# refresh-bio/vclust

Measured on AMD Instinct MI355X. Metric: genome pairs/sec through prefilter+align (ani.tsv), higher is better.
Workload: dtype u64

## Files before the change

### vclust_amd/build.py

```python
import os
import pathlib
import shutil
import subprocess
import sys

PKG_DIR = pathlib.Path(__file__).resolve().parent
ROOT = PKG_DIR.parent
CSRC = PKG_DIR / 'csrc'
LIB_PATH = PKG_DIR / 'libvclust_gpu.so'
ORACLE_DIR = ROOT / 'oracle'

SOURCES = ['vg_core.cpp', 'vg_genomes.cpp', 'vg_inflate.cpp', 'vg_io.cpp', 'vg_api.cpp', 'vg_synth.cpp', 'vg_prefilter.hip', 'vg_align.hip', 'vg_dist.hip', 'vg_cluster.hip', 'vg_dedup.hip']


def _hipcc() -> str:
    for cand in (os.environ.get('HIPCC'), shutil.which('hipcc'), '/opt/rocm/bin/hipcc'):
        if cand and pathlib.Path(cand).exists():
            return cand
    raise RuntimeError('hipcc not found (needs ROCm)')


def _stale(target: pathlib.Path, deps) -> bool:
    if not target.exists():
        return True
    t = target.stat().st_mtime
    return any(pathlib.Path(d).stat().st_mtime > t for d in deps)


def build_lib(force: bool = False, verbose: bool = False) -> pathlib.Path:
    srcs = [CSRC / s for s in SOURCES]
    deps = srcs + [CSRC / 'vg_common.h', ROOT / 'include' / 'vclust_gpu.h']
    if not force and not _stale(LIB_PATH, deps):
        return LIB_PATH
    obj_dir = PKG_DIR / '_obj'
    obj_dir.mkdir(exist_ok=True)
    hipcc = _hipcc()
    flags = ['--offload-arch=gfx950', '-O3', '-std=c++17', '-fPIC', '-Wall', '-Wno-unused-function',
             '-Wno-unused-result', f'-I{ROOT / "include"}']
    if os.environ.get('VG_LINES') == '1':
        flags.append('-gline-tables-only')
    if os.environ.get('VG_DEV') == '1':
        flags.append('-DVG_DEV_KERNELS')
    objs = []
    procs = []
    for s in srcs:
        o = obj_dir / (s.name + '.o')
        objs.append(o)
        if force or _stale(o, [s, CSRC / 'vg_common.h', ROOT / 'include' / 'vclust_gpu.h']):
            cmd = [hipcc, *flags, '-x', 'hip', '-c', str(s), '-o', str(o)]
            if verbose:
                print(' '.join(cmd), file=sys.stderr)
            procs.append((s, subprocess.Popen(cmd, stdout=subprocess.PIPE, stderr=subprocess.STDOUT, text=True)))
    for s, p in procs:
        out, _ = p.communicate()
        if p.returncode != 0:
            raise RuntimeError(f'hipcc failed on {s.name}:\n{out}')
        if verbose and out.strip():
            print(out, file=sys.stderr)
    cmd = [hipcc, '--offload-arch=gfx950', '-shared', '-fPIC', '-o', str(LIB_PATH), *map(str, objs), '-lz', '-lpthread', '-ldl']
    r = subprocess.run(cmd, stdout=subprocess.PIPE, stderr=subprocess.STDOUT, text=True)
    if r.returncode != 0:
        raise RuntimeError(f'link failed:\n{r.stdout}')
    return LIB_PATH


def build_oracle(verbose: bool = False) -> pathlib.Path:
    r = subprocess.run(['make', '-C', str(ORACLE_DIR)], stdout=subprocess.PIPE, stderr=subprocess.STDOUT, text=True)
    if r.returncode != 0:
        raise RuntimeError(f'oracle build failed:\n{r.stdout}')
    if verbose:
        print(r.stdout, file=sys.stderr)
    return ORACLE_DIR / '_build' / 'liboracle.so'


if __name__ == '__main__':
    force = '--force' in sys.argv
    print(build_lib(force=force, verbose=True))
    print(build_oracle(verbose=False))
```

### vclust_amd/csrc/vg_align.hip

```cpp
#include "vg_common.h"
#include <rocprim/rocprim.hpp>
#include <algorithm>
#include <numeric>
#include <cstring>
#include <memory>
#include <mutex>
#include <optional>

namespace {

constexpr int RR_PAD = 128;

struct ref_desc {
    int64_t rr_w;
    int64_t mask_w;
    int64_t stab;
    int64_t sent;
    int32_t L;
    int32_t n_rr;
    int32_t genome;
    int32_t has_n;
    int32_t pos_bits;
    int32_t tag_bits;
};

struct lz_dev_params { int mal, msl, mrd, mqd, reg, aw, am, ar; int ablate; int pw_after, pw_miss; int weak_ratio; int margin; int seed_choice; };


__device__ __forceinline__ uint32_t loadm32(const uint32_t* __restrict__ mk, int64_t p) {
    int64_t w = p >> 5; int sh = (int)(p & 31);
    uint64_t m = (uint64_t)mk[w] | ((uint64_t)mk[w + 1] << 32);
    return (uint32_t)(m >> sh);
}
__device__ __forceinline__ uint32_t squeeze16(uint32_t x) {
    x &= 0x55555555u;
    x = (x | (x >> 1)) & 0x33333333u;
    x = (x | (x >> 2)) & 0x0F0F0F0Fu;
    x = (x | (x >> 4)) & 0x00FF00FFu;
    return (x | (x >> 8)) & 0x0000FFFFu;
}
__device__ __forceinline__ uint32_t squeeze(uint64_t x) {
    return squeeze16((uint32_t)x) | (squeeze16((uint32_t)(x >> 32)) << 16);
}
struct planes32 { uint32_t lo, hi; };
__device__ __forceinline__ planes32 planes_of(uint64_t codes) { return { squeeze(codes), squeeze(codes >> 1) }; }

__device__ __forceinline__ planes32 loadp(const uint32_t* __restrict__ pl, int64_t p) {
    const uint32_t off = ((uint32_t)p >> 5) << 3; const uint32_t sh = (uint32_t)p & 31u;
    uint4 v; __builtin_memcpy(&v, (const char*)pl + off, 16);
    asm volatile("" :: "v"(v.w));
    return { __builtin_amdgcn_alignbit(v.z, v.x, sh), __builtin_amdgcn_alignbit(v.w, v.y, sh) };
}
__device__ __forceinline__ uint32_t diff32(const planes32 a, const planes32 b) { return (a.lo ^ b.lo) | (a.hi ^ b.hi); }
__device__ __forceinline__ uint32_t slots(int lo, int hi) {
    if (lo < 0) lo = 0; if (hi > 32) hi = 32;
    if (hi <= lo) return 0u;
    const uint32_t a = (hi == 32) ? ~0u : ((1u << hi) - 1u);
    return a & ~((1u << lo) - 1u);
}

struct pair_ctx {
    const uint32_t* qpl; const uint32_t* qmk; int qlen; int q_has_n;
    const uint32_t* rpl; const uint32_t* rmk; int n_rr; int L; int r_has_n;
};

__device__ __forceinline__ uint32_t mism32(const pair_ctx& c, int qp, int rp, int rlo, int rhi) {
    const int lo = max(-qp, rlo - rp); const int hi = min(c.qlen - qp, rhi - rp);
    if (lo <= 0 && hi >= 32) {
        uint32_t mm = diff32(loadp(c.qpl, qp), loadp(c.rpl, rp));
        if (c.q_has_n) mm |= loadm32(c.qmk, qp);
        if (c.r_has_n) mm |= loadm32(c.rmk, rp);
        return mm;
    }
    const uint32_t ok = slots(lo, hi);
    if (ok == 0) return ~0u;
    const int qs = qp < 0 ? 0 : qp, rs = rp < 0 ? 0 : rp;
    planes32 xq = loadp(c.qpl, qs), xr = loadp(c.rpl, rs);
    if (qp < 0) { xq.lo <<= -qp; xq.hi <<= -qp; }
    if (rp < 0) { xr.lo <<= -rp; xr.hi <<= -rp; }
    uint32_t mm = diff32(xq, xr);
    if (c.q_has_n) { uint32_t sp = loadm32(c.qmk, qs); if (qp < 0) sp <<= -qp; mm |= sp; }
    if (c.r_has_n) { uint32_t sp = loadm32(c.rmk, rs); if (rp < 0) sp <<= -rp; mm |= sp; }
    return mm | ~ok;
}
__device__ __forceinline__ int strand_lo(const pair_ctx& c, int rp) { return rp > c.L ? c.L + 1 : 0; }
__device__ __forceinline__ int strand_hi(const pair_ctx& c, int rp) { return rp > c.L ? c.n_rr : c.L; }

__device__ __forceinline__ int match_len_lane(const pair_ctx& c, int qp, int rp, int cap) {
    int l = 0;
    while (l < cap) {
        const uint32_t mm = mism32(c, qp + l, rp + l, strand_lo(c, rp), strand_hi(c, rp));
        if (mm) return l + __builtin_ctz(mm);
        l += 32;
    }
    return l;
}

__device__ __forceinline__ int match_len32_q(const pair_ctx& c, const planes32 xq, uint32_t qbad, int rp) {
    uint32_t mm = diff32(xq, loadp(c.rpl, rp)) | qbad;
    if (c.r_has_n) mm |= loadm32(c.rmk, rp);
    const int hi = c.n_rr - rp; if (hi < 32) mm |= ~slots(0, hi);
    const int sj = c.L - rp; if ((unsigned)sj < 32u) mm |= 1u << sj;
    return mm ? __builtin_ctz(mm) : 32;
}

__device__ __forceinline__ uint32_t lane32(uint32_t v, int src_lane) { return (uint32_t)__builtin_amdgcn_readlane((int)v, src_lane); }
__device__ __forceinline__ uint32_t lane_prev32(uint32_t v) {
    return (uint32_t)__builtin_amdgcn_update_dpp(0, (int)v, 0x138, 0xf, 0xf, false);
}
__device__ __forceinline__ int wave_sum(int v) {
    int t = 0;
#pragma unroll
    for (int b = 0; b < 6; ++b) t += __popcll(__ballot((v >> b) & 1)) << b;
    return t;
}

__device__ __forceinline__ uint32_t extend_mask0(const pair_ctx& c, int qp, int rp, int dir, int bound, int lane, int rlo, int rhi) {
    uint32_t mm = ~0u;
    const int e0 = 32 * lane;
    if (e0 < bound) {
        if (dir > 0) mm = mism32(c, qp + e0, rp + e0, rlo, rhi);
        else mm = __brev(mism32(c, qp - e0 - 32, rp - e0 - 32, rlo, rhi));
        const int rem = bound - e0; if (rem < 32) mm |= ~slots(0, rem);
    }
    return mm;
}

__device__ __forceinline__ int extend(const pair_ctx& c, const lz_dev_params& P, int qp, int rp, int dir, int bound,
                                      int lane, int* n_match, uint32_t mm_first, int rlo, int rhi) {
    int accepted = 0, matches_total = 0;
    int first_mm = -1;
    uint32_t carry_mm = 0;
    uint32_t carry_ok = 0;
    int base = 0;
    int cum_before = 0;
    const uint32_t awmask = (P.aw >= 32) ? ~0u : ((1u << P.aw) - 1u);
    if (bound <= 0) { *n_match = 0; return 0; }
    for (;;) {
        uint32_t mm = mm_first;
        if (base > 0) {
            mm = ~0u;
            const int e0 = base + 32 * lane;
            if (e0 < bound) {
                if (dir > 0) mm = mism32(c, qp + e0, rp + e0, rlo, rhi);
                else mm = __brev(mism32(c, qp - e0 - 32, rp - e0 - 32, rlo, rhi));
                const int rem = bound - e0; if (rem < 32) mm |= ~slots(0, rem);
            }
        }
        const unsigned long long anyb = __ballot(mm != 0);
        if (first_mm < 0 && anyb) {
            const int fl = __builtin_ctzll(anyb);
            first_mm = base + 32 * fl + __builtin_ctz(lane32(mm, fl));
        }
        uint32_t prev_mm = lane_prev32(mm); const uint32_t okb = ~mm; uint32_t prev_ok = lane_prev32(okb);
        if (lane == 0) { prev_mm = carry_mm; prev_ok = carry_ok; }
        int viol = 32;
        {
            const uint32_t tail = (P.aw > 1) ? (prev_mm >> (32 - (P.aw - 1))) : 0u;
            if ((int)(__popc(mm) + __popc(tail)) > P.am) {
                uint32_t bits = mm;
                for (int skip = P.am - (int)__popc(tail); skip > 0; --skip) bits &= bits - 1;
                while (bits) {
                    const int j = __builtin_ctz(bits);
                    const uint32_t hi = (j == 31) ? mm : (mm & ((2u << j) - 1u));
                    int cnt;
                    if (j + 1 >= P.aw) cnt = __popc(hi & (awmask << (j + 1 - P.aw)));
                    else cnt = __popc(hi) + __popc(prev_mm >> (32 - (P.aw - 1 - j)));
                    if (cnt > P.am) { viol = j; break; }
                    bits &= bits - 1;
                }
            }
        }
        const unsigned long long vb = __ballot(viol < 32);
        if (anyb) {
            uint32_t run = okb;
            for (int t = 1; t < P.ar; ++t) run &= __builtin_amdgcn_alignbit(okb, prev_ok, (uint32_t)(32 - t));
            const int fv = vb ? __builtin_ctzll(vb) : 64;
            const int vj = (int)lane32((uint32_t)viol, fv & 63);
            uint32_t cand = run;
            if (lane > fv) cand = 0;
            else if (lane == fv) cand &= (vj == 0) ? 0u : ((1u << vj) - 1u);
            const unsigned long long cb = __ballot(cand != 0);
            if (cb) {
                const int hl = 63 - __builtin_clzll(cb);
                const uint32_t ch = lane32(cand, hl); const uint32_t mh = lane32(mm, hl);
                const int hj = 31 - __builtin_clz(ch);
                accepted = base + 32 * hl + hj + 1;
                int tot = wave_sum(lane < hl ? 32 - __popc(mm) : 0);
                const uint32_t upto = (hj == 31) ? ~0u : ((2u << hj) - 1u);
                tot += (hj + 1) - __popc(mh & upto);
                matches_total = cum_before + tot;
            }
        } else {
            accepted = base + 2048; matches_total = cum_before + 2048;
        }
        if (vb) break;
        if (base + 2048 >= bound) break;
        cum_before += anyb ? wave_sum(32 - __popc(mm)) : 2048;
        carry_mm = lane32(mm, 63); carry_ok = lane32(okb, 63);
        base += 2048;
    }
    if (first_mm < 0) first_mm = bound;
    if (first_mm > bound) first_mm = bound;
    if (accepted < first_mm) { accepted = first_mm; matches_total = first_mm; }
    if (accepted > bound) { accepted = bound; }
    *n_match = matches_total;
    return accepted;
}

__device__ __forceinline__ uint64_t low_bits64(int n) { return n >= 64 ? ~0ULL : (n <= 0 ? 0ULL : ((1ULL << n) - 1)); }

__device__ __forceinline__ int gap_score(const pair_ctx& c, int i, int g, int pred0, int E, int lane, int rlo, int rhi,
                                         int* pm_out, int* sm_out) {
    const int reflen = E - pred0;
    const int skip = (reflen >= 0 && g > reflen) ? g - reflen : 0;
    const int q0 = i - g;
    uint32_t ok_o = 0, ok_n = 0;
    {
        const int e0 = 32 * lane;
        if (e0 < g) {
            const uint32_t in = (g - e0 >= 32) ? 0xffffffffu : ((1u << (g - e0)) - 1u);
            ok_o = ~mism32(c, q0 + e0, pred0 + e0, rlo, rhi) & in;
            ok_n = ~mism32(c, q0 + e0, E - g + e0, rlo, rhi) & in;
        }
    }
    int tot_n = 0;
    for (int w2 = 0; 32 * w2 < g; ++w2) tot_n += __popc(lane32(ok_n, w2));
    int best_v = -1, best_pm = 0, best_sm = 0;
    const int nbits = 32 - __builtin_clz((unsigned)g | 1u);
    int po = 0;
    const int n_split = g - skip;
    for (int w = 0; 64 * w <= n_split; ++w) {
        const uint64_t O = (uint64_t)lane32(ok_o, 2 * w) | ((uint64_t)lane32(ok_o, (2 * w + 1) & 63) << 32);
        const int a = 64 * w + lane;
        const int s0 = 64 * w + skip;
        const int ws = s0 >> 6;
        const uint64_t N0 = (uint64_t)lane32(ok_n, (2 * ws) & 63) | ((uint64_t)lane32(ok_n, (2 * ws + 1) & 63) << 32);
        const uint64_t N1 = (uint64_t)lane32(ok_n, (2 * ws + 2) & 63) | ((uint64_t)lane32(ok_n, (2 * ws + 3) & 63) << 32);
        int pn0 = 0;
        for (int w2 = 0; w2 < 2 * ws && 32 * w2 < g; ++w2) pn0 += __popc(lane32(ok_n, w2));
        const int pn1 = pn0 + __popcll(N0);
        const int sp = s0 + lane;
        const bool second = (sp >> 6) > ws;
        const int before = second ? pn1 + __popcll(N1 & low_bits64(sp & 63)) : pn0 + __popcll(N0 & low_bits64(sp & 63));
        const int pre = po + __popcll(O & low_bits64(lane));
        const int suf = tot_n - before;
        const bool valid = a <= n_split;
        const int v = pre + suf;
        unsigned long long act = __ballot(valid);
        if (act) {
            for (int b = nbits - 1; b >= 0; --b) {
                const unsigned long long m = __ballot(valid && ((v >> b) & 1)) & act;
                if (m) act = m;
            }
            const int wl = 63 - __builtin_clzll(act);
            const int vmax = (int)lane32((uint32_t)v, wl);
            if (vmax >= best_v) { best_v = vmax; best_pm = (int)lane32((uint32_t)pre, wl); best_sm = (int)lane32((uint32_t)suf, wl); }
        }
        po += __popcll(O);
    }
    *pm_out = best_pm; *sm_out = best_sm;
    return best_pm + best_sm;
}

__device__ __forceinline__ void rr_chunk_planes(const uint32_t* __restrict__ gpl, const uint32_t* __restrict__ gmk, int L, int64_t ch,
                                                uint32_t* lo_out, uint32_t* hi_out, uint32_t* mask_out) {
    const int64_t p0 = ch * 32;
    uint32_t lo = 0, hi = 0, mask = 0xffffffffu;
    const int64_t nf = (int64_t)L - p0;
    if (nf > 0) {
        const uint32_t xl = gpl[2 * ch], xh = gpl[2 * ch + 1], m = gmk[ch];
        if (nf >= 32) { lo = xl; hi = xh; mask = m; }
        else { const uint32_t lowm = (1u << nf) - 1u; lo = xl & lowm; hi = xh & lowm; mask = (m & lowm) | ~lowm; }
    }
    const int64_t jlo = (L + 1 - p0) > 0 ? (L + 1 - p0) : 0;
    const int64_t jhi = (2 * (int64_t)L - p0) < 31 ? (2 * (int64_t)L - p0) : 31;
    if (jlo <= jhi) {
        const int64_t fstart = 2 * (int64_t)L - p0 - 31;
        planes32 x; uint32_t m;
        if (fstart >= 0) { x = loadp(gpl, fstart); m = loadm32(gmk, fstart); }
        else { x = loadp(gpl, 0); x.lo <<= -fstart; x.hi <<= -fstart; m = loadm32(gmk, 0) << (-fstart); }
        const uint32_t rl = ~__brev(x.lo), rh = ~__brev(x.hi), mr = __brev(m);
        const uint32_t hi1 = (jhi == 31) ? 0xffffffffu : ((1u << (jhi + 1)) - 1);
        const uint32_t lo1 = (jlo == 0) ? 0u : ((1u << jlo) - 1);
        const uint32_t sl1 = hi1 & ~lo1;
        lo |= rl & sl1; hi |= rh & sl1;
        mask = (mask & ~sl1) | (mr & sl1);
    }
    *lo_out = lo & ~mask; *hi_out = hi & ~mask; *mask_out = mask;
}

__device__ __forceinline__ uint32_t bucket_of(uint32_t xl, uint32_t xh, int msl) { const uint32_t m = (1u << msl) - 1u; return (xl & m) | ((xh & m) << msl); }
__device__ __forceinline__ uint32_t tag_of(uint32_t xl, uint32_t xh, int msl, int tag_bits) {
    const int tl = (tag_bits + 1) >> 1, th = tag_bits >> 1;
    return ((xl >> msl) & ((1u << tl) - 1u)) | (((xh >> msl) & ((1u << th) - 1u)) << tl);
}

constexpr int LDS_TAB = 16384;
constexpr int LDS_STAGE = 22016;
constexpr int TOP_BITS = 9;
constexpr int BIG_RR = 131072;
__device__ __forceinline__ void lds_sync() { asm volatile("s_waitcnt lgkmcnt(0)\n\ts_barrier" ::: "memory"); }

__device__ __forceinline__ uint32_t wave_scan_inclusive(uint32_t v) {
    v += (uint32_t)__builtin_amdgcn_update_dpp(0, (int)v, 0x111, 0xf, 0xf, true);
    v += (uint32_t)__builtin_amdgcn_update_dpp(0, (int)v, 0x112, 0xf, 0xf, true);
    v += (uint32_t)__builtin_amdgcn_update_dpp(0, (int)v, 0x114, 0xf, 0xf, true);
    v += (uint32_t)__builtin_amdgcn_update_dpp(0, (int)v, 0x118, 0xf, 0xf, true);
    v += (uint32_t)__builtin_amdgcn_update_dpp(0, (int)v, 0x142, 0xa, 0xf, false);
    v += (uint32_t)__builtin_amdgcn_update_dpp(0, (int)v, 0x143, 0xc, 0xf, false);
    return v;
}
// ... 616 lines not shown
                    }
                    const unsigned long long at = chunk_base + (kk & (RCHUNK - 1));
                    if (lane == 0 && at < arena_cap) {
                        region_rec rg; rg.task = tk.out_idx; rg.qstart = r_qstart; rg.qend = r_qend;
                        rg.rstart = r_rstart; rg.rend = r_rend; rg.n_match = r_match; rg.k = kk; rg.t = (uint32_t)t;
                        arena[at] = rg;
                    }
                }
            }
            in_region = false;
        }
    };

    for (int phase = 0; phase < (S > 1 ? 2 : 1); ++phase) {
    while (i < phase_end) {
        const int qi = i + lane;
        int best_len = 0, best_pos = 0; bool hit_close = false;
        if (qi < lim && lane < pw) {
            const bool alive_l = alive && (lit + lane <= P.mqd);
            const int pred_l = pred + lane;
            const planes32 xq = loadp(c.qpl, qi);
            bool q_ok_a = true, q_ok_s = (qi + P.msl <= c.qlen);
            uint32_t qbad = (c.qlen - qi < 32) ? ~slots(0, c.qlen - qi) : 0u;
            if (c.q_has_n) {
                const uint32_t m = loadm32(c.qmk, qi);
                q_ok_a = (m & ((1u << P.mal) - 1u)) == 0;
                q_ok_s = q_ok_s && (m & ((1u << P.msl) - 1u)) == 0;
                qbad |= m;
            }
            const bool do_a = q_ok_a && !(ABL & 16);
            const bool do_s = alive_l && q_ok_s && !(ABL & 1);
            uint32_t s_u = 0, s_e = 0;
            const uint32_t posmask = (rd.pos_bits >= 32) ? 0xffffffffu : ((1u << rd.pos_bits) - 1u);
            const uint32_t qtag = tag_of(xq.lo, xq.hi, P.msl, rd.tag_bits);
            const bool probing = (do_a || do_s) && q_ok_s;
            const uint32_t b = bucket_of(xq.lo, xq.hi, P.msl);
            uint4 f0 = make_uint4(~0u, ~0u, ~0u, ~0u), f1 = f0;
            if (FUSED) {
                if (probing) { const uint32_t* sl = fslots + ((size_t)tk.r_slot * FUSED_SLOTS + b) * 8; __builtin_memcpy(&f0, sl, 16); __builtin_memcpy(&f1, sl + 4, 16); }
            } else if (probing) {
                uint2 bb; __builtin_memcpy(&bb, stab + (b ? b - 1 : 0u), 8);
                s_u = b ? bb.x : 0u; s_e = b ? bb.y : bb.x;
            }
            const int pred0 = pred - lit;
            const bool pred_rc = pred0 > c.L;
            const int win_lo = pred0;
            const int win_hi = pred_rc ? pred_l + P.mrd - 1 : min(pred_l + P.mrd - 1, c.L - 1);
            int sbest_len = 0, sbest_pos = 0, sbest_ad = 0, ncap_a = 0, ncap_s = 0;
            const uint32_t win_span = (uint32_t)(win_hi - win_lo);
            const bool win_any = win_hi >= win_lo;
            auto scan4 = [&](const uint4 v, const unsigned vm) {
                const uint32_t e4[4] = { v.x, v.y, v.z, v.w };
                unsigned am = 0, sm = 0;
#pragma unroll
                for (int j = 0; j < 4; ++j) {
                    const uint32_t ps = e4[j] & posmask;
                    am |= (uint32_t)(rd.tag_bits == 0 || (e4[j] >> rd.pos_bits) == qtag) << j;
                    sm |= (uint32_t)(ps - (uint32_t)win_lo <= win_span) << j;
                }
                am &= do_a ? vm : 0u; sm &= (do_s && win_any) ? vm : 0u;
                unsigned cm = am | sm;
                while (cm) {
                    const int j = __builtin_ctz(cm); cm &= cm - 1;
                    const uint32_t ej = j == 0 ? e4[0] : j == 1 ? e4[1] : j == 2 ? e4[2] : e4[3];
                    const int rp = (int)(ej & posmask);
                    const int l0 = match_len32_q(c, xq, qbad, rp);
                    if ((am >> j) & 1u) {
                        int l = l0;
                        if (l >= P.mal) {
                            if (l >= 32) {
                                if (ncap_a++ > 0 || best_len >= 32) {
                                    l = match_len_lane(c, qi, rp, 1 << 30);
                                    if (best_len == 32) best_len = match_len_lane(c, qi, best_pos, 1 << 30);
                                }
                            }
                            if (l > best_len || (l == best_len && rp < best_pos)) { best_len = l; best_pos = rp; }
                        }
                    }
                    if ((sm >> j) & 1u) {
                        int l = l0;
                        if (l >= P.msl) {
                            if (l >= 32) {
                                if (ncap_s++ > 0 || sbest_len >= 32) {
                                    l = match_len_lane(c, qi, rp, 1 << 30);
                                    if (sbest_len == 32) sbest_len = match_len_lane(c, qi, sbest_pos, 1 << 30);
                                }
                            }
                            const int ad = abs(rp - pred_l);
                            const bool better = P.seed_choice == 1 ? (sbest_len == 0 || ad < sbest_ad || (ad == sbest_ad && (l > sbest_len || (l == sbest_len && rp < sbest_pos))))
                                                                   : (l > sbest_len || (l == sbest_len && (ad < sbest_ad || (ad == sbest_ad && rp < sbest_pos))));
                            if (better) { sbest_len = l; sbest_pos = rp; sbest_ad = ad; }
                        }
                    }
                }
            };
            if (FUSED) {
                if (DEV) { ++n_ab; }
                const unsigned vm0 = (unsigned)(!(f0.x >> 31)) | ((unsigned)(!(f0.y >> 31)) << 1) | ((unsigned)(!(f0.z >> 31)) << 2) | ((unsigned)(!(f0.w >> 31)) << 3);
                const unsigned vm1 = (unsigned)(!(f1.x >> 31)) | ((unsigned)(!(f1.y >> 31)) << 1) | ((unsigned)(!(f1.z >> 31)) << 2) | ((unsigned)(!(f1.w >> 31)) << 3);
                if (vm0) scan4(f0, vm0);
                if (vm1) scan4(f1, vm1);
                if ((f1.w >> 31) && f1.w != ~0u) {
                    s_u = f1.w & 0x7fffffu; const uint32_t cnt = (f1.w >> 23) & 0xffu;
                    if (cnt == 255u) { uint2 bb; __builtin_memcpy(&bb, stab + (b ? b - 1 : 0u), 8); s_e = b ? bb.y : bb.x; }
                    else s_e = s_u + cnt;
                }
                const unsigned long long hit0 = __ballot(best_len > 0 || sbest_len > 0);
                if (hit0 && lane > __builtin_ctzll(hit0)) s_u = s_e;
            }
            while (s_u < s_e) {
                if (DEV) { ++n_ab; }
                uint4 v; __builtin_memcpy(&v, sent + s_u, 16);
                const uint32_t left = s_e - s_u;
                scan4(v, left >= 4u ? 0xfu : ((1u << left) - 1u));
                s_u += 4;
                const unsigned long long hit = __ballot(best_len > 0 || sbest_len > 0);
                if (hit && lane > __builtin_ctzll(hit)) s_u = s_e;
            }
            if (best_len > 0 && sbest_len > 0 && best_pos != sbest_pos && best_len >= 32 && sbest_len + P.margin + 1 > 32) {
                if (best_len == 32) best_len = match_len_lane(c, qi, best_pos, 1 << 30);
                if (sbest_len == 32) sbest_len = match_len_lane(c, qi, sbest_pos, 1 << 30);
            }
            if (best_len > 0 && (sbest_len == 0 || best_len > sbest_len + P.margin - ((P.weak_ratio > 0 && lit + lane > P.weak_ratio * sbest_len) ? 1 : 0))) {
                const int d = best_pos - pred_l;
                hit_close = alive_l && ((best_pos > c.L) == pred_rc) && d >= -P.mrd && d <= P.mrd;
            } else if (sbest_len > 0) { best_len = sbest_len; best_pos = sbest_pos; hit_close = true; }
        }
        const unsigned long long hb = __ballot(best_len > 0);
        if (DEV) ++n_iter;
        PROF_MARK(0);
        if (!hb) {
            const int n = min(pw, lim - i);
            i += n; lit += n; if (alive) { pred += n; if (lit > P.mqd) alive = false; }
            pw = pw < P.pw_miss ? P.pw_miss : 64;
            continue;
        }
        const int f = __builtin_ctzll(hb);
        pw = P.pw_after;
        if (!(ABL & 64)) {
            ++n_events;
            if (n_events == 24) __builtin_amdgcn_s_setprio(1);
            else if (n_events == 64) __builtin_amdgcn_s_setprio(2);
            else if (n_events == 160) __builtin_amdgcn_s_setprio(3);
        }
        const int ev_pos = (int)lane32((uint32_t)best_pos, f);
        const bool ev_close = lane32((uint32_t)hit_close, f) != 0;
        i += f; lit += f; if (alive) { pred += f; if (lit > P.mqd) alive = false; }
        const int gap_end_ref = pred - 1;
        const int ev_i = i;
        const int ev_len = (int)lane32((uint32_t)best_len, f);
        const int rlo = strand_lo(c, ev_pos), rhi = strand_hi(c, ev_pos);
        const int kept_after = (in_region && r_qend - r_qstart + 1 >= P.reg) ? r_qend + 1 : kept_end;
        const int bwd_bound = ev_close ? 0 : i - kept_after;
        const uint32_t mm_b = (!ev_close && !(ABL & 2)) ? extend_mask0(c, i, ev_pos, -1, bwd_bound, lane, rlo, rhi) : ~0u;
        const uint32_t mm_f = extend_mask0(c, i, ev_pos, +1, 1 << 30, lane, rlo, rhi);
        PROF_MARK(1);
        if (!ev_close) {
            close_region();
            int bm = 0;
            const int b = (ABL & 2) ? 0 : extend(c, P, i, ev_pos, -1, bwd_bound, lane, &bm, mm_b, rlo, rhi);
            r_qstart = i - b; r_rstart = ev_pos - b; r_match = bm; r_rend = -1;
            in_region = true;
        }
        PROF_MARK(2);
        int fe, fm = 0;
        {
            fe = (ABL & 4) ? P.mal : extend(c, P, i, ev_pos, +1, 1 << 30, lane, &fm, mm_f, rlo, rhi);
            r_match += fm;
        }
        if (ev_close) {
            int pm = 0, sm = 0;
            if (lit > 0 && !(ABL & 8)) {
                int xl = ev_len;
                if (xl >= 32) {
                    const unsigned long long mb = __ballot(mm_f != 0);
                    xl = mb ? 32 * __builtin_ctzll(mb) + __builtin_ctz(lane32(mm_f, __builtin_ctzll(mb))) : 2048;
                    if (xl >= 2048) xl = match_len_lane(c, i, ev_pos, 1 << 30);
                }
                r_match += gap_score(c, i, lit, pred - lit, ev_pos + xl, lane, rlo, rhi, &pm, &sm);
            }
            const int tru = gap_end_ref + 1, vir = vend + lit - pm;
            vend = max(tru, vir) - sm + (fe - fm);
            r_rend = max(r_rend, max(ev_pos + fe - 1, vend - 1));
            r_rstart = min(r_rstart, ev_pos);
        }
        i += fe; pred = ev_pos + fe; lit = 0; alive = true;
        if (!ev_close) { r_rend = pred - 1; vend = pred; }
        PROF_MARK(3);
        r_qend = i - 1;
        if (S > 1) {
            const bool span_ok = i - r_qstart >= P.reg;
            if (phase == 1) {
                const int v = min(S - 1, ev_i / seg_len);
                if (v != look_v) { look_v = v; look_cur = 0; }
                const seg_rec* lg = s_log + v * SEG_LOG_CAP; const int nv = s_cnt[v];
                while (look_cur < nv && lg[look_cur].i_ev < ev_i) ++look_cur;
                if (span_ok && look_cur < nv && lg[look_cur].i_ev == ev_i && lg[look_cur].ev_pos == ev_pos && (lg[look_cur].VN >> 31)) {
                    synced = true; sync_v = v; sync_idx = look_cur;
                    M += (uint32_t)r_match; A -= (uint32_t)r_qstart;
                    break;
                }
            } else if (log_n < SEG_LOG_CAP) {
                if (lane == 0) {
                    seg_rec rc; rc.i_ev = ev_i; rc.ev_pos = ev_pos;
                    rc.VM = M + (uint32_t)r_match; rc.VA = A - (uint32_t)r_qstart; rc.VN = NR | (span_ok ? 0x80000000u : 0u);
                    s_log[w * SEG_LOG_CAP + log_n] = rc;
                }
                ++log_n;
            }
        }
    }
    if (S > 1 && phase == 0) {
        if (lane == 0) s_cnt[w] = log_n;
        __syncthreads();
        phase_end = lim;
    }
    if (synced) break;
    }
    if (!synced) close_region();
    if (S > 1) {
        if (lane == 0) { s_end[w][0] = M; s_end[w][1] = A; s_end[w][2] = NR; s_sync_v[w] = sync_v; s_sync_idx[w] = sync_idx; }
        __syncthreads();
        if (threadIdx.x == 0) {
            uint32_t tm = 0, ta = 0, tn = 0, bm = 0, ba = 0, bn = 0; int cur = 0;
            for (;;) {
                tm += s_end[cur][0] - bm; ta += s_end[cur][1] - ba; tn += s_end[cur][2] - bn;
                const int v = s_sync_v[cur];
                if (v < 0) break;
                const seg_rec rc = s_log[v * SEG_LOG_CAP + s_sync_idx[cur]];
                bm = rc.VM; ba = rc.VA; bn = rc.VN & 0x7fffffffu; cur = v;
            }
            vg_pair_stat st; st.n_match = tm; st.aln_len = ta; st.n_regions = tn;
            stats[tk.out_idx] = st;
        }
        return;
    }
    if (prof) { M = (uint32_t)(pc[psel] >> 4); A = (uint32_t)n_events; }
    if (ABL & 1024) {
        int mab = n_ab, msb = n_sb;
        for (int o = 32; o; o >>= 1) { mab = max(mab, __shfl_xor(mab, o)); msb = max(msb, __shfl_xor(msb, o)); }
        M = (uint32_t)n_iter; A = (uint32_t)n_events; if (ABL & 2048) { M = (uint32_t)mab; A = (uint32_t)msb; }
    }
    if (ABL & (32 | 1024)) NR = (uint32_t)((long long)wall_clock64() - t_start);
    if (REG && (NR & (RCHUNK - 1)) != 0) {
        const uint32_t used = NR & (RCHUNK - 1);
        const unsigned long long at = chunk_base + used + (uint32_t)lane;
        if (used + (uint32_t)lane < (uint32_t)RCHUNK && at < arena_cap) arena[at].task = ~0u;
    }
    if (lane == 0) { vg_pair_stat st; st.n_match = M; st.aln_len = A; st.n_regions = NR; stats[tk.out_idx] = st; }
}

#define PARSE_KERNEL(NAME, S, DEV, WAVES, FAST, REG, ...) \
    __global__ void __launch_bounds__(256) __attribute__((amdgpu_waves_per_eu(WAVES, 8))) NAME(PARSE_ARGS) { \
        lz_parse_body<S, DEV, FAST, REG, ##__VA_ARGS__>(PARSE_ARG_NAMES); }
PARSE_KERNEL(k_lz_parse, 1, false, 8, false, false)
PARSE_KERNEL(k_lz_parse_fast, 1, false, 8, true, false)
PARSE_KERNEL(k_lz_parse_seg, 4, false, 8, false, false)
PARSE_KERNEL(k_lz_parse_seg_fast, 4, false, 8, true, false)
PARSE_KERNEL(k_lz_parse_regions, 1, false, 8, false, true)
PARSE_KERNEL(k_lz_parse_fast_regions, 1, false, 8, true, true)
PARSE_KERNEL(k_lz_parse_fast_fused, 1, false, 8, true, false, true)
__global__ void __launch_bounds__(256)
k_index_fuse(const ref_desc* __restrict__ refs, int first_ref, int n_refs, const uint32_t* __restrict__ stab_pool, const uint32_t* __restrict__ sent_pool,
             uint32_t* __restrict__ fslots) {
    for (int r = blockIdx.x; r < n_refs; r += gridDim.x) {
        const ref_desc rd = refs[first_ref + r];
        const uint32_t* stab = stab_pool + rd.stab; const uint32_t* sent = sent_pool + rd.sent;
        uint32_t* out = fslots + (size_t)(first_ref + r) * FUSED_SLOTS * 8;
        for (int b = threadIdx.x; b < FUSED_SLOTS; b += blockDim.x) {
            const uint32_t lo = b ? stab[b - 1] : 0u, hi = stab[b], n = hi - lo;
            uint32_t w[8];
#pragma unroll
            for (int j = 0; j < 8; ++j) w[j] = (uint32_t)j < n ? sent[lo + j] : ~0u;
            if (n > 8) w[7] = 0x80000000u | (((n - 7) < 255u ? (n - 7) : 255u) << 23) | (lo + 7);
            uint4 a = make_uint4(w[0], w[1], w[2], w[3]), c2 = make_uint4(w[4], w[5], w[6], w[7]);
            __builtin_memcpy(out + (size_t)b * 8, &a, 16); __builtin_memcpy(out + (size_t)b * 8 + 4, &c2, 16);
        }
    }
}
#ifdef VG_DEV_KERNELS
PARSE_KERNEL(k_lz_parse_dev, 1, true, 3, false, false)
#endif

__global__ void __launch_bounds__(256)
k_region_counts(const task_dev* __restrict__ tasks, int64_t n_tasks, const vg_pair_stat* __restrict__ stats, unsigned long long* __restrict__ cnt) {
    for (int64_t t = (int64_t)blockIdx.x * blockDim.x + threadIdx.x; t <= n_tasks; t += (int64_t)gridDim.x * blockDim.x)
        cnt[t] = t < n_tasks ? (unsigned long long)stats[tasks[t].out_idx].n_regions : 0ULL;
}
__global__ void __launch_bounds__(256)
k_regions_place(const region_rec* __restrict__ arena, unsigned long long n_slots, const unsigned long long* __restrict__ first,
                unsigned long long n_out, vg_region* __restrict__ out, unsigned int* __restrict__ bad) {
    for (unsigned long long i = (unsigned long long)blockIdx.x * blockDim.x + threadIdx.x; i < n_slots; i += (unsigned long long)gridDim.x * blockDim.x) {
        const region_rec r = arena[i];
        if (r.task == ~0u) continue;
        const unsigned long long at = first[r.t] + r.k;
        if (at >= first[r.t + 1] || at >= n_out) { atomicAdd(bad, 1u); continue; }
        vg_region o; o.task = r.task; o.qstart = r.qstart; o.qend = r.qend; o.rstart = r.rstart; o.rend = r.rend; o.n_match = r.n_match;
        out[at] = o;
    }
}

inline int grid_for(int64_t n, int block = 256, int max_blocks = 256 * 16) {
    int64_t b = (n + block - 1) / block; if (b < 1) b = 1;
    return (int)std::min<int64_t>(b, max_blocks);
}

}

static std::mutex g_fit_mu;
static bool g_fit_set = false;
static vg_lz_fit g_fit{ 3, -1, 3 };
static vg_lz_fit lz_fit_now() {
    std::lock_guard<std::mutex> lk(g_fit_mu);
    if (!g_fit_set) {
        g_fit_set = true;
        if (const char* e = vg_dev_getenv("VG_LZ_WEAK_SEED")) if (*e) g_fit.weak_seed_ratio = atoi(e);
        if (const char* e = vg_dev_getenv("VG_LZ_ANCHOR_MARGIN")) if (*e) g_fit.anchor_margin = atoi(e);
        if (const char* e = vg_dev_getenv("VG_LZ_SEED_CHOICE")) if (*e) g_fit.seed_choice = atoi(e);
        if (g_fit.weak_seed_ratio != 3 || g_fit.anchor_margin >= 0 || g_fit.seed_choice != 3)
            fprintf(stderr, "libvclust_gpu: LZ fit constants changed by developer switches (weak seed ratio %d, anchor margin %d, seed choice %d): results differ from the reference's\n",
// ... 636 lines not shown
```

Measured before the change: 2.550 million.

## Add fast extension path with wide mismatch loads and bit-sliced window check

```diff
diff --git a/vclust_amd/build.py b/vclust_amd/build.py
--- a/vclust_amd/build.py
+++ b/vclust_amd/build.py
@@ -29,7 +29,7 @@
 
 def build_lib(force: bool = False, verbose: bool = False) -> pathlib.Path:
     srcs = [CSRC / s for s in SOURCES]
-    deps = srcs + [CSRC / 'vg_common.h', ROOT / 'include' / 'vclust_gpu.h']
+    deps = srcs + [CSRC / 'vg_common.h', CSRC / 'vg_window.h', ROOT / 'include' / 'vclust_gpu.h']
     if not force and not _stale(LIB_PATH, deps):
         return LIB_PATH
     obj_dir = PKG_DIR / '_obj'
@@ -46,7 +46,7 @@
     for s in srcs:
         o = obj_dir / (s.name + '.o')
         objs.append(o)
-        if force or _stale(o, [s, CSRC / 'vg_common.h', ROOT / 'include' / 'vclust_gpu.h']):
+        if force or _stale(o, [s, CSRC / 'vg_common.h', CSRC / 'vg_window.h', ROOT / 'include' / 'vclust_gpu.h']):
             cmd = [hipcc, *flags, '-x', 'hip', '-c', str(s), '-o', str(o)]
             if verbose:
                 print(' '.join(cmd), file=sys.stderr)
diff --git a/vclust_amd/csrc/vg_align.hip b/vclust_amd/csrc/vg_align.hip
--- a/vclust_amd/csrc/vg_align.hip
+++ b/vclust_amd/csrc/vg_align.hip
@@ -1,4 +1,5 @@
 #include "vg_common.h"
+#include "vg_window.h"
 #include <rocprim/rocprim.hpp>
 #include <algorithm>
 #include <numeric>
@@ -115,9 +116,22 @@
     return t;
 }
 
-__device__ __forceinline__ uint32_t extend_mask0(const pair_ctx& c, int qp, int rp, int dir, int bound, int lane, int rlo, int rhi) {
+template <bool UNI>
+__device__ __forceinline__ uint32_t extend_mask(const pair_ctx& c, int qp, int rp, int dir, int base, int bound, int lane, int rlo, int rhi) {
+    if (UNI && base + 2048 <= bound) {
+        const int q0 = dir > 0 ? qp + base : qp - base - 2048, r0 = dir > 0 ? rp + base : rp - base - 2048;
+        if (q0 >= 0 && q0 + 2048 <= c.qlen && r0 >= rlo && r0 + 2048 <= rhi) {
+            const uint32_t off = (uint32_t)(dir > 0 ? lane : 63 - lane) * 8u;
+            const char* qrow = (const char*)c.qpl + (size_t)(q0 >> 5) * 8; const char* rrow = (const char*)c.rpl + (size_t)(r0 >> 5) * 8;
+            const uint32_t qsh = (uint32_t)q0 & 31u, rsh = (uint32_t)r0 & 31u;
+            uint4 vq, vr; __builtin_memcpy(&vq, qrow + off, 16); __builtin_memcpy(&vr, rrow + off, 16);
+            const uint32_t mm = (__builtin_amdgcn_alignbit(vq.z, vq.x, qsh) ^ __builtin_amdgcn_alignbit(vr.z, vr.x, rsh)) |
+                                (__builtin_amdgcn_alignbit(vq.w, vq.y, qsh) ^ __builtin_amdgcn_alignbit(vr.w, vr.y, rsh));
+            return dir > 0 ? mm : __brev(mm);
+        }
+    }
     uint32_t mm = ~0u;
-    const int e0 = 32 * lane;
+    const int e0 = base + 32 * lane;
     if (e0 < bound) {
         if (dir > 0) mm = mism32(c, qp + e0, rp + e0, rlo, rhi);
         else mm = __brev(mism32(c, qp - e0 - 32, rp - e0 - 32, rlo, rhi));
@@ -125,7 +139,12 @@
     }
     return mm;
 }
-
+template <bool UNI>
+__device__ __forceinline__ uint32_t extend_mask0(const pair_ctx& c, int qp, int rp, int dir, int bound, int lane, int rlo, int rhi) {
+    return extend_mask<UNI>(c, qp, rp, dir, 0, bound, lane, rlo, rhi);
+}
+
+template <bool FAST>
 __device__ __forceinline__ int extend(const pair_ctx& c, const lz_dev_params& P, int qp, int rp, int dir, int bound,
                                       int lane, int* n_match, uint32_t mm_first, int rlo, int rhi) {
     int accepted = 0, matches_total = 0;
@@ -138,15 +157,7 @@
     if (bound <= 0) { *n_match = 0; return 0; }
     for (;;) {
         uint32_t mm = mm_first;
-        if (base > 0) {
-            mm = ~0u;
-            const int e0 = base + 32 * lane;
-            if (e0 < bound) {
-                if (dir > 0) mm = mism32(c, qp + e0, rp + e0, rlo, rhi);
-                else mm = __brev(mism32(c, qp - e0 - 32, rp - e0 - 32, rlo, rhi));
-                const int rem = bound - e0; if (rem < 32) mm |= ~slots(0, rem);
-            }
-        }
+        if (base > 0) mm = extend_mask<FAST>(c, qp, rp, dir, base, bound, lane, rlo, rhi);
         const unsigned long long anyb = __ballot(mm != 0);
         if (first_mm < 0 && anyb) {
             const int fl = __builtin_ctzll(anyb);
@@ -157,7 +168,9 @@
         int viol = 32;
         {
             const uint32_t tail = (P.aw > 1) ? (prev_mm >> (32 - (P.aw - 1))) : 0u;
-            if ((int)(__popc(mm) + __popc(tail)) > P.am) {
+            if ((int)(__popc(mm) + __popc(tail)) > P.am && FAST) {
+                viol = vg_first_violation_15_7(mm, prev_mm);
+            } else if ((int)(__popc(mm) + __popc(tail)) > P.am) {
                 uint32_t bits = mm;
                 for (int skip = P.am - (int)__popc(tail); skip > 0; --skip) bits &= bits - 1;
                 while (bits) {
@@ -1080,20 +1093,20 @@
         const int rlo = strand_lo(c, ev_pos), rhi = strand_hi(c, ev_pos);
         const int kept_after = (in_region && r_qend - r_qstart + 1 >= P.reg) ? r_qend + 1 : kept_end;
         const int bwd_bound = ev_close ? 0 : i - kept_after;
-        const uint32_t mm_b = (!ev_close && !(ABL & 2)) ? extend_mask0(c, i, ev_pos, -1, bwd_bound, lane, rlo, rhi) : ~0u;
-        const uint32_t mm_f = extend_mask0(c, i, ev_pos, +1, 1 << 30, lane, rlo, rhi);
+        const uint32_t mm_b = (!ev_close && !(ABL & 2)) ? extend_mask0<FAST>(c, i, ev_pos, -1, bwd_bound, lane, rlo, rhi) : ~0u;
+        const uint32_t mm_f = extend_mask0<FAST>(c, i, ev_pos, +1, 1 << 30, lane, rlo, rhi);
         PROF_MARK(1);
         if (!ev_close) {
             close_region();
             int bm = 0;
-            const int b = (ABL & 2) ? 0 : extend(c, P, i, ev_pos, -1, bwd_bound, lane, &bm, mm_b, rlo, rhi);
+            const int b = (ABL & 2) ? 0 : extend<FAST>(c, P, i, ev_pos, -1, bwd_bound, lane, &bm, mm_b, rlo, rhi);
             r_qstart = i - b; r_rstart = ev_pos - b; r_match = bm; r_rend = -1;
             in_region = true;
         }
         PROF_MARK(2);
         int fe, fm = 0;
         {
-            fe = (ABL & 4) ? P.mal : extend(c, P, i, ev_pos, +1, 1 << 30, lane, &fm, mm_f, rlo, rhi);
+            fe = (ABL & 4) ? P.mal : extend<FAST>(c, P, i, ev_pos, +1, 1 << 30, lane, &fm, mm_f, rlo, rhi);
             r_match += fm;
         }
         if (ev_close) {
diff --git a/vclust_amd/csrc/vg_window.h b/vclust_amd/csrc/vg_window.h
--- /dev/null
+++ b/vclust_amd/csrc/vg_window.h
@@ -0,0 +1,40 @@
+#pragma once
+#include <stdint.h>
+
+#if defined(__HIPCC__) || defined(__HIP__)
+#define VG_HD __host__ __device__ __forceinline__
+#else
+#define VG_HD inline
+#endif
+
+VG_HD uint32_t vg_sh64(uint32_t hi, uint32_t lo, int t) {
+    return (uint32_t)((((uint64_t)hi << 32) | lo) >> (32 - t));
+}
+VG_HD void vg_fa(uint32_t a, uint32_t b, uint32_t c, uint32_t& s, uint32_t& cy) { s = a ^ b ^ c; cy = (a & b) | (c & (a ^ b)); }
+VG_HD uint32_t vg_maj(uint32_t a, uint32_t b, uint32_t c) { return (a & b) | (c & (a ^ b)); }
+
+VG_HD uint32_t vg_window_over_15_7(uint32_t mm, uint32_t prev_mm) {
+    uint32_t c[15];
+    c[0] = mm;
+#if defined(__HIP_DEVICE_COMPILE__)
+#pragma unroll
+    for (int t = 1; t < 15; ++t) c[t] = __builtin_amdgcn_alignbit(mm, prev_mm, (uint32_t)(32 - t));
+#else
+    for (int t = 1; t < 15; ++t) c[t] = vg_sh64(mm, prev_mm, t);
+#endif
+    uint32_t s1[5], c2[7];
+#pragma unroll
+    for (int k = 0; k < 5; ++k) vg_fa(c[3 * k], c[3 * k + 1], c[3 * k + 2], s1[k], c2[k]);
+    uint32_t s;
+    vg_fa(s1[0], s1[1], s1[2], s, c2[5]);
+    c2[6] = vg_maj(s1[3], s1[4], s);
+    uint32_t t0, t1, c4a, c4b;
+    vg_fa(c2[0], c2[1], c2[2], t0, c4a);
+    vg_fa(c2[3], c2[4], c2[5], t1, c4b);
+    const uint32_t c4c = vg_maj(c2[6], t0, t1);
+    return vg_maj(c4a, c4b, c4c);
+}
+VG_HD int vg_first_violation_15_7(uint32_t mm, uint32_t prev_mm) {
+    const uint32_t v = vg_window_over_15_7(mm, prev_mm) & mm;
+    return v ? __builtin_ctz(v) : 32;
+}
```

After: 2.610 million, median of 6. 2.3% higher.
